# xkuubix/MonteCarlo-Gated-MIL

Measured on AMD Instinct MI355X. Metric: bags/sec × MCDO-samples (T=100) at N=2048,d=512; 1/2/4/8-GPU + %HBM roofline, higher is better.
Workload: dtype bf16

## Files before the change

montecarlo-gated-mil_amd/csrc/mcgmil_fused.hip:

```cpp
#define MCGMIL_KERNELS_TEMPLATES_ONLY
#include "../../include/mcgmil.h"
#include "mcgmil_kernels.h"
#include "mcgmil_error.h"
#include "mcgmil_fused.h"


namespace mcgmil {

__global__ __launch_bounds__(1024) void plan_regions_kernel(const int32_t* bag_off, int B, int T,
                                                            int cap, int32_t* region_off) {
    __shared__ int part[1024];
    const int tid = threadIdx.x;
    const int per = (B + 1023) / 1024;
    const int b0 = tid * per, b1 = b0 + per < B ? b0 + per : B;
    int sum = 0;
    for (int b = b0; b < b1; ++b) {
        const int ts = region_t_groups(bag_off[b + 1] - bag_off[b], T, cap);
        sum += (T + ts - 1) / ts;
    }
    part[tid] = sum;
    __syncthreads();
    for (int o = 1; o < 1024; o <<= 1) {
        const int v = tid >= o ? part[tid - o] : 0;
        __syncthreads();
        part[tid] += v;
        __syncthreads();
    }
    int run = part[tid] - sum;
    for (int b = b0; b < b1; ++b) {
        region_off[b] = run;
        const int ts = region_t_groups(bag_off[b + 1] - bag_off[b], T, cap);
        run += (T + ts - 1) / ts;
    }
    if (tid == 1023) region_off[B] = part[1023];
}

}

namespace mcgmil_detail {

long long fused_regions(const mcgmil::GateParams& gp, long long total_rows, int cap, bool estimate) {
    if (gp.uniform_rows > 0) {
        const int ts = mcgmil::region_t_groups(gp.uniform_rows, gp.T, cap);
        return (long long)gp.B * ((gp.T + ts - 1) / ts);
    }
    if (estimate) return (long long)gp.T * total_rows / cap;
    return (2ll * gp.T * total_rows + cap - 1) / cap + gp.B + 1;
}

namespace {

template <typename E, int PPW, int MAXC, bool ONE>
int launch(const mcgmil::GateParams& gp, long long total_rows, hipStream_t s) {
    auto* k = gp.clock ? &mcgmil::gate_fused_kernel<E, PPW, MAXC, ONE, true>
                       : &mcgmil::gate_fused_kernel<E, PPW, MAXC, ONE>;
    if (int rc = raise_lds_limit(reinterpret_cast<const void*>(k), "gate_fused_kernel LDS limit")) return rc;
    constexpr int cap = mcgmil::fused_cap<MAXC>();
    if (gp.uniform_rows <= 0) {
        hipLaunchKernelGGL(mcgmil::plan_regions_kernel, dim3(1), dim3(1024), 0, s, gp.bag_off, gp.B,
                           gp.T, cap, const_cast<int32_t*>(gp.region_off));
        hipError_t e = hipGetLastError();
        if (e != hipSuccess) return hip_fail(e, "plan_regions_kernel launch");
    }
    const long long grid = fused_regions(gp, total_rows, cap, false);
    if (grid == 0) return MCGMIL_OK;
    if (grid > 0x7fffffffll) return fail(MCGMIL_E_UNSUPPORTED, "too many regions for one launch");
    const size_t lds = mcgmil::fused_kernel_lds_bytes<E, MAXC>(gp.L);
    if (lds > 160 * 1024) return fail(MCGMIL_E_UNSUPPORTED, "fused kernel: L too large for its LDS");
    hipLaunchKernelGGL(k, dim3((unsigned)grid), dim3(mcgmil::kGateThreads), lds, s, gp);
    hipError_t e = hipGetLastError();
    return e == hipSuccess ? MCGMIL_OK : hip_fail(e, "gate_fused_kernel launch");
}

template <typename E, int MAXC>
int launch_maxc(const mcgmil::GateParams& gp, int ppw, bool one, long long total_rows, hipStream_t s) {
    if (ppw == 1) return one ? launch<E, 1, MAXC, true>(gp, total_rows, s) : launch<E, 1, MAXC, false>(gp, total_rows, s);
    return one ? launch<E, 2, MAXC, true>(gp, total_rows, s) : launch<E, 2, MAXC, false>(gp, total_rows, s);
}

}

int launch_gate_fused(const mcgmil::GateParams& gp, bool bf16, int ppw, int maxc, bool one,
                      long long total_rows, hipStream_t s) {
    if (bf16) return maxc == 2 ? launch_maxc<__bf16, 2>(gp, ppw, one, total_rows, s)
                               : launch_maxc<__bf16, 4>(gp, ppw, one, total_rows, s);
    return maxc == 2 ? launch_maxc<float, 2>(gp, ppw, one, total_rows, s)
                     : launch_maxc<float, 4>(gp, ppw, one, total_rows, s);
}

}
```

montecarlo-gated-mil_amd/csrc/mcgmil_kernels.h:

```cpp
#pragma once
#include "mcgmil_device.h"

namespace mcgmil {

struct GateParams {
    const void* H;
    long long ldh;
    const int32_t* bag_off;
    int B, T, L, D, C, G, P;
    long long total_samples;
    const void* Wp;
    uint32_t wp_bytes;
    const float* bv;
    const float* bu;
    const float* wa;
    const float* ba;
    float sf, sa;
    uint32_t thr_f, thr_a;
    uint32_t thrx_f;
    uint32_t k0, k1;
    uint32_t bag_base;
    int t_base;
    const uint32_t* bag_ids;
    const int32_t* tile_bag;
// ... 51 lines not shown
        Nb = p.uniform_rows;
        if (narrow) {
            const uint32_t r = (uint32_t)R, pb = (uint32_t)per_bag;
            bag = (int)(r / pb);
            const uint32_t local = r - (uint32_t)bag * pb;
            t = (int)(local / (uint32_t)Nb);
            n = (int)(local - (uint32_t)t * (uint32_t)Nb);
        } else {
            bag = (int)(R / per_bag);
            const long long local = R - (long long)bag * per_bag;
            t = (int)(local / Nb);
            n = (int)(local - (long long)t * Nb);
        }
        hrow = bag * Nb + n;
    } else if (R < p.total_samples) {
        if (p.tile_bag) {
            bag = p.tile_bag[R0 / BM];
            while ((long long)p.T * p.bag_off[bag + 1] <= R) ++bag;
        } else {
            bag = find_bag(p.bag_off, p.B, p.T, R);
        }
        const int ob = p.bag_off[bag];
        Nb = p.bag_off[bag + 1] - ob;
        const long long local = R - (long long)p.T * ob;
        if (narrow) {
            t = (int)((uint32_t)local / (uint32_t)Nb);
            n = (int)((uint32_t)local - (uint32_t)t * (uint32_t)Nb);
        } else {
            t = (int)(local / Nb);
            n = (int)(local - (long long)t * Nb);
        }
        hrow = ob + n;
    }
    int* ri = rinfo + kRowInfo * tid;
    ri[0] = hrow; ri[1] = t; ri[2] = n; ri[3] = bag; ri[4] = Nb;
    ri[5] = (int)(p.bag_ids ? p.bag_ids[bag] : p.bag_base + (uint32_t)bag);
}

#ifndef MCGMIL_KERNELS_TEMPLATES_ONLY
__global__ void plan_tiles_kernel(const int32_t* bag_off, int B, int T, long long total_samples,
                                  int BM, long long tiles, int32_t* tile_bag) {
    const long long i = (long long)blockIdx.x * blockDim.x + threadIdx.x;
    if (i >= tiles) return;
    const long long R = i * BM;
    tile_bag[i] = R < total_samples ? find_bag(bag_off, B, T, R) : 0;
}
#endif

__device__ __forceinline__ float gated_product_scaled(float ax, float by) {
    ax = fminf(fmaxf(ax, -43.280851226668903f), 43.280851226668903f);
    const float a = __builtin_amdgcn_exp2f(ax);
    const float b = __builtin_amdgcn_exp2f(by);
    const float ia = 1.0f + a;
    return (1.0f - a) * __builtin_amdgcn_rcpf(fmaf(ia, b, ia));
}

#ifndef MCGMIL_DIAG
#define MCGMIL_DIAG 0
#endif
#ifndef MCGMIL_PHILOX_ROUNDS
#define MCGMIL_PHILOX_ROUNDS 10
#endif

constexpr float kM2Log2e = -2.8853900817779268f;
constexpr float kMLog2e = -1.4426950408889634f;

struct HeadVec { f32x4 bv, bu, wa; };

template <int PPW>
__device__ __forceinline__ void load_head_vectors(const GateParams& p, int q0, int lane,
                                                  HeadVec (&hv)[PPW]) {
    const int DB = p.D >> 4;
#pragma unroll
    for (int jp = 0; jp < PPW; ++jp) {
        const int q = q0 + jp < p.P ? q0 + jp : p.P - 1;
        const int g = q / DB, db = q - g * DB;
        const int d0 = db * 16 + 4 * (lane >> 4);
        hv[jp].bv = *reinterpret_cast<const f32x4*>(p.bv + (size_t)g * p.D + d0) * kM2Log2e;
        hv[jp].bu = *reinterpret_cast<const f32x4*>(p.bu + (size_t)g * p.D + d0) * kMLog2e;
        hv[jp].wa = *reinterpret_cast<const f32x4*>(p.wa + (size_t)g * p.D + d0);
    }
}

template <int RT, int PPW, int MAXC, bool ONE_CLASS, int RTV = RT>
__device__ __forceinline__ void fold_pairs(const GateParams& p, const f32x4 (&acc)[RT][2 * PPW],
                                           int q0, int lane, float (&part)[MAXC][RT],
                                           const HeadVec* pre = nullptr) {
    const int DB = p.D >> 4;
    const float av_s = p.sf * kM2Log2e, au_s = p.sf * kMLog2e;
#pragma unroll
    for (int jp = 0; jp < PPW; ++jp) {
        const int q = q0 + jp;
        if (q >= p.P) break;
        const int g = q / DB, db = q - g * DB;
        const int d0 = db * 16 + 4 * (lane >> 4);
        f32x4 bvv, buv;
        f32x4 coef[MAXC];
        if (ONE_CLASS && pre) {
            bvv = pre[jp].bv;
            buv = pre[jp].bu;
            coef[0] = pre[jp].wa;
#pragma unroll
            for (int c = 1; c < MAXC; ++c) coef[c] = f32x4{0.f, 0.f, 0.f, 0.f};
        } else {
            bvv = *reinterpret_cast<const f32x4*>(p.bv + (size_t)g * p.D + d0);
            buv = *reinterpret_cast<const f32x4*>(p.bu + (size_t)g * p.D + d0);
            bvv *= kM2Log2e;
            buv *= kMLog2e;
#pragma unroll
            for (int c = 0; c < MAXC; ++c) {
                const int cc = ONE_CLASS ? g : c;
                const bool use = ONE_CLASS ? (c == 0) : ((c < p.C) && (p.G == 1 || c == g));
                const f32x4 w = *reinterpret_cast<const f32x4*>(p.wa + (size_t)(use ? cc : 0) * p.D + d0);
                coef[c] = use ? w : f32x4{0.f, 0.f, 0.f, 0.f};
            }
        }
#pragma unroll
        for (int rt = 0; rt < RTV; ++rt) {
#pragma unroll
            for (int v = 0; v < 4; ++v) {
                const float ax = fmaf(acc[rt][2 * jp][v], av_s, bvv[v]);
                const float by = fmaf(acc[rt][2 * jp + 1][v], au_s, buv[v]);
                if constexpr (ONE_CLASS) {
#if MCGMIL_DIAG & 8
                    part[0][rt] = fmaf(fmaf(ax, coef[0][v], by), ax, part[0][rt]);
                    continue;
#endif
                    const float a = __builtin_amdgcn_exp2f(fminf(fmaxf(ax, -43.280851226668903f),
                                                                 43.280851226668903f));
                    const float b = __builtin_amdgcn_exp2f(by);
                    const float ia = 1.0f + a;
                    const float r = __builtin_amdgcn_rcpf(fmaf(ia, b, ia));
                    part[0][rt] = fmaf(fmaf(-a, coef[0][v], coef[0][v]), r, part[0][rt]);
                } else {
                    const float pr = gated_product_scaled(ax, by);
#pragma unroll
                    for (int c = 0; c < MAXC; ++c) part[c][rt] = fmaf(pr, coef[c][v], part[c][rt]);
                }
            }
        }
    }
}

template <int BM, int MAXC>
__host__ __device__ constexpr int red_floats() { return kGateWaves * MAXC * 4 * BM; }

template <int BM, int MAXC, int ROWS = 16>
__device__ __forceinline__ void finish_scores(const GateParams& p, long long R0,
                                              float (&part)[MAXC][BM / ROWS], f32x4 zacc,
                                              bool zwave, float* red, float* zred,
                                              const int* rinfo, int one_class, int waves_per_gate,
                                              bool have_keep, bool keep, float* lg_out,
                                              float* z_out, long long obase) {
    constexpr int RT = BM / ROWS;
    constexpr int NG = 64 / ROWS;
    const int tid = threadIdx.x, lane = tid & 63, wave = tid >> 6;
    const int ncls = one_class < 0 ? MAXC : 1;
#pragma unroll
    for (int c = 0; c < MAXC; ++c) {
        if (c >= ncls) break;
        const int cls = one_class < 0 ? c : one_class;
        if (cls >= MAXC) break;
        float* dst = red + ((size_t)(wave * MAXC + cls) * NG + lane / ROWS) * BM + (lane % ROWS);
#pragma unroll
        for (int q = 0; q < RT; ++q) dst[ROWS * q] = part[c][q];
    }
    if (zwave && lane < 16) {
#pragma unroll
        for (int c = 0; c < MAXC; ++c) zred[c * BM + wave * 16 + lane] = zacc[c];
    }
    MCGMIL_STAMP(p, 5);
    __syncthreads();
    MCGMIL_STAMP(p, 6);
    const int r = wave * 16 + (lane & 15), c = lane >> 4;
    if (r >= BM || c >= p.C) return;
    const int* ri = rinfo + kRowInfo * r;
    if (ri[0] < 0) return;
    float s = 0.f;
    const int nw = waves_per_gate ? waves_per_gate : kGateWaves;
    for (int k = 0; k < nw; ++k) {
        const int w = waves_per_gate ? c * waves_per_gate + k : k;
        const float* src = red + (size_t)(w * MAXC + c) * NG * BM + r;
#pragma unroll
        for (int g = 0; g < NG; ++g) s += src[g * BM];
    }
    s += p.ba[c];
    const int t = ri[1], n = ri[2], bag = ri[3], Nb = ri[4];
    if (p.keep_att) {
        const size_t abase = (size_t)p.T * p.C * (size_t)p.bag_off[bag];
        keep = p.keep_att[abase + ((size_t)t * p.C + c) * Nb + n] != 0;
    } else if (!have_keep) {
        keep = attention_keep(p.k0, p.k1, (uint32_t)ri[5], (uint32_t)(p.t_base + t), (uint32_t)c,
                              (uint32_t)n, p.thr_a);
    }
    const size_t o = (size_t)(R0 + r - obase) * p.C + c;
    lg_out[o] = s * (keep ? p.sa : 0.f);
    z_out[o] = zred[c * BM + r] * p.sf;
}

constexpr int kSoftmaxRows = 16;

#ifndef MCGMIL_NT_A
#define MCGMIL_NT_A 1
#endif
__device__ __forceinline__ void store_a(float* dst, float v) {
#if MCGMIL_NT_A
    __builtin_nontemporal_store(v, dst);
#else
    *dst = v;
#endif
}

__device__ __forceinline__ void softmax_group(int ltid, bool active, int Nb, int C, const float* lg,
                                              const float* zz, float* Ao, float* Yo, float* sred) {
    const int tid = ltid, lane = ltid & 63, wave = ltid >> 6;
    if (Nb == 0) {
        if (active && tid < C) Yo[tid] = 0.f;
        return;
    }
    const int Nl = active ? Nb : 0;
    if (C == 2 && Nb <= 256 * kSoftmaxRows) {
        float (*sred2)[4] = reinterpret_cast<float (*)[4]>(sred);
        float e0[kSoftmaxRows], e1[kSoftmaxRows];
        float2 zr[kSoftmaxRows];
        float m0 = -INFINITY, m1 = -INFINITY;
#pragma unroll
        for (int k = 0; k < kSoftmaxRows; ++k) {
            const int n = tid + 256 * k;
            float2 l = make_float2(-INFINITY, -INFINITY);
            zr[k] = make_float2(0.f, 0.f);
            if (n < Nl) {
                l = *reinterpret_cast<const float2*>(lg + (size_t)n * 2);
                zr[k] = *reinterpret_cast<const float2*>(zz + (size_t)n * 2);
            }
            e0[k] = l.x;
            e1[k] = l.y;
            m0 = fmaxf(m0, e0[k]);
            m1 = fmaxf(m1, e1[k]);
        }
        m0 = wave_max(m0);
        m1 = wave_max(m1);
        if (lane == 0) { sred2[0][wave] = m0; sred2[1][wave] = m1; }
        __syncthreads();
        m0 = fmaxf(fmaxf(sred2[0][0], sred2[0][1]), fmaxf(sred2[0][2], sred2[0][3]));
        m1 = fmaxf(fmaxf(sred2[1][0], sred2[1][1]), fmaxf(sred2[1][2], sred2[1][3]));
        __syncthreads();
        float s0 = 0.f, y0 = 0.f, s1 = 0.f, y1 = 0.f;
#pragma unroll
        for (int k = 0; k < kSoftmaxRows; ++k) {
            const int n = tid + 256 * k;
            if (n < Nl) {
                const float2 z = zr[k];
                e0[k] = expf(e0[k] - m0);
                e1[k] = expf(e1[k] - m1);
                s0 += e0[k];
                s1 += e1[k];
                y0 = fmaf(e0[k], z.x, y0);
                y1 = fmaf(e1[k], z.y, y1);
            }
        }
        s0 = wave_sum(s0);
        y0 = wave_sum(y0);
        s1 = wave_sum(s1);
        y1 = wave_sum(y1);
        if (lane == 0) {
            sred2[0][wave] = s0; sred2[1][wave] = y0; sred2[2][wave] = s1; sred2[3][wave] = y1;
        }
        __syncthreads();
        s0 = (sred2[0][0] + sred2[0][1]) + (sred2[0][2] + sred2[0][3]);
        y0 = (sred2[1][0] + sred2[1][1]) + (sred2[1][2] + sred2[1][3]);
        s1 = (sred2[2][0] + sred2[2][1]) + (sred2[2][2] + sred2[2][3]);
        y1 = (sred2[3][0] + sred2[3][1]) + (sred2[3][2] + sred2[3][3]);
        __syncthreads();
        const float inv0 = 1.0f / s0, inv1 = 1.0f / s1;
        if (Ao) {
            float* Ao1 = Ao + Nb;
#pragma unroll
            for (int k = 0; k < kSoftmaxRows; ++k) {
// ... 101 lines not shown
template <> struct Raw<__bf16> { uint4 v; };
template <> struct Raw<float> { f32x4 lo, hi; };
__device__ __forceinline__ Raw<__bf16> load_raw(const __bf16* p) {
    Raw<__bf16> r; r.v = *reinterpret_cast<const uint4*>(p); return r;
}
__device__ __forceinline__ Raw<float> load_raw(const float* p) {
    Raw<float> r;
    r.lo = *reinterpret_cast<const f32x4*>(p);
    r.hi = *reinterpret_cast<const f32x4*>(p + 4);
    return r;
}
__device__ __forceinline__ void store_masked(const Raw<__bf16>& h, uint32_t kb, __bf16* dst) {
    uint4 v = h.v;
    v.x &= ((kb & 1u) ? 0x0000FFFFu : 0u) | ((kb & 2u) ? 0xFFFF0000u : 0u);
    v.y &= ((kb & 4u) ? 0x0000FFFFu : 0u) | ((kb & 8u) ? 0xFFFF0000u : 0u);
    v.z &= ((kb & 16u) ? 0x0000FFFFu : 0u) | ((kb & 32u) ? 0xFFFF0000u : 0u);
    v.w &= ((kb & 64u) ? 0x0000FFFFu : 0u) | ((kb & 128u) ? 0xFFFF0000u : 0u);
    *reinterpret_cast<uint4*>(dst) = v;
}
__device__ __forceinline__ void store_masked(const Raw<float>& h, uint32_t kb, float* dst) {
    f32x4 a = h.lo, b = h.hi;
    a.x = (kb & 1u) ? a.x : 0.f;   a.y = (kb & 2u) ? a.y : 0.f;
    a.z = (kb & 4u) ? a.z : 0.f;   a.w = (kb & 8u) ? a.w : 0.f;
    b.x = (kb & 16u) ? b.x : 0.f;  b.y = (kb & 32u) ? b.y : 0.f;
    b.z = (kb & 64u) ? b.z : 0.f;  b.w = (kb & 128u) ? b.w : 0.f;
    *reinterpret_cast<f32x4*>(dst) = a;
    *reinterpret_cast<f32x4*>(dst + 4) = b;
}

__device__ __forceinline__ void store_dropped(const Raw<__bf16>& h, uint4 o, uint32_t thrx,
                                              uint32_t inval, __bf16* dst) {
    uint4 v = h.v;
    v.x = __builtin_amdgcn_bitop3_b32(v.x, drop_mask16x2_flipped(o.x, thrx), inval, 0x10);
    v.y = __builtin_amdgcn_bitop3_b32(v.y, drop_mask16x2(o.y, thrx), inval, 0x10);
    v.z = __builtin_amdgcn_bitop3_b32(v.z, drop_mask16x2_flipped(o.z, thrx), inval, 0x10);
    v.w = __builtin_amdgcn_bitop3_b32(v.w, drop_mask16x2(o.w, thrx), inval, 0x10);
    *reinterpret_cast<uint4*>(dst) = v;
}
__device__ __forceinline__ uint32_t keep_lo(uint32_t m) { return ~(uint32_t)((int32_t)(m << 16) >> 16); }
__device__ __forceinline__ uint32_t keep_hi(uint32_t m) { return ~(uint32_t)((int32_t)m >> 16); }
__device__ __forceinline__ void store_dropped(const Raw<float>& h, uint4 o, uint32_t thrx,
                                              uint32_t inval, float* dst) {
    const uint32_t m0 = drop_mask16x2_flipped(o.x, thrx) | inval, m1 = drop_mask16x2(o.y, thrx) | inval;
    const uint32_t m2 = drop_mask16x2_flipped(o.z, thrx) | inval, m3 = drop_mask16x2(o.w, thrx) | inval;
    f32x4 a = h.lo, b = h.hi;
    a.x = __uint_as_float(__float_as_uint(a.x) & keep_lo(m0));
    a.y = __uint_as_float(__float_as_uint(a.y) & keep_hi(m0));
    a.z = __uint_as_float(__float_as_uint(a.z) & keep_lo(m1));
    a.w = __uint_as_float(__float_as_uint(a.w) & keep_hi(m1));
    b.x = __uint_as_float(__float_as_uint(b.x) & keep_lo(m2));
    b.y = __uint_as_float(__float_as_uint(b.y) & keep_hi(m2));
    b.z = __uint_as_float(__float_as_uint(b.z) & keep_lo(m3));
    b.w = __uint_as_float(__float_as_uint(b.w) & keep_hi(m3));
    *reinterpret_cast<f32x4*>(dst) = a;
    *reinterpret_cast<f32x4*>(dst + 4) = b;
}

constexpr int kPipeBM = 128;
#ifndef MCGMIL_VPM
#define MCGMIL_VPM 2
#endif
constexpr int VPM = MCGMIL_VPM;
#ifndef MCGMIL_SCHED
#define MCGMIL_SCHED 0
#endif
constexpr int HD = 2;
template <typename E>
__host__ __device__ constexpr int pipe_slots() { return 2; }

template <typename E, int MAXC>
__host__ __device__ constexpr size_t pipe_lds_bytes() {
    return (size_t)pipe_slots<E>() * kPipeBM * 32 * sizeof(E) + (size_t)red_floats<kPipeBM, MAXC>() * 4 +
           (size_t)MAXC * kPipeBM * 4 + (size_t)kRowInfo * kPipeBM * 4;
}

template <typename E>
__device__ __forceinline__ void load_classifier_lds(__amdgpu_buffer_rsrc_t wrs, uint32_t zsoff, int KS, E* zw) {
    for (int i = threadIdx.x; i < KS * 64; i += kGateThreads)
        *reinterpret_cast<f32x4*>(zw + (size_t)i * 8) = __builtin_bit_cast(
            f32x4, __builtin_amdgcn_raw_buffer_load_b128(wrs, (uint32_t)i * 8u * (uint32_t)sizeof(E), zsoff, 0));
}

template <typename E, int PPW, int MAXC, bool REPLAY, bool ONE_CLASS, bool EARLY_HV = true,
          bool ZL = false, bool ZLOAD = true, int RTV = kPipeBM / 16>
__device__ __forceinline__ void pipe_tile(const GateParams& p, long long R0, E* Xs, float* red,
                                          float* zred, const int* rinfo, float* lg_out,
                                          float* z_out, long long obase, E* zw = nullptr) {
    constexpr int BM = kPipeBM;
    constexpr int RT = BM / 16;
    constexpr int NJ = 2 * PPW;
    constexpr int SLOT = RT * 64 * 8;
    const int tid = threadIdx.x, lane = tid & 63, wave = tid >> 6;
    const int KS = p.L >> 5;

    const int* ri = rinfo + kRowInfo * (wave * 16 + (lane & 15));
    const int hrow = ri[0];
    const bool valid = hrow >= 0;
    const int kq = lane >> 4;
    const E* hsrc = reinterpret_cast<const E*>(p.H) + (size_t)(valid ? hrow : 0) * p.ldh + kq * 8;
    const uint32_t cn = (uint32_t)ri[2], ct = (uint32_t)(p.t_base + ri[1]), cb = (uint32_t)ri[5];
    const uint8_t* kfe = REPLAY ? p.keep_feat + (size_t)(valid ? R0 + wave * 16 + (lane & 15) : 0) *
                                                    (p.L >> 3) + kq
                                : nullptr;

    const uint32_t inval = valid ? 0u : 0xFFFFFFFFu;
    auto stage = [&](int s, const Raw<E>& h, E* slot) {
        if constexpr (REPLAY) {
            const uint32_t kb = kfe[(size_t)(s < KS ? s : KS - 1) * 4];
            store_masked(h, kb & ~inval, slot + tid * 8);
        } else {
#if MCGMIL_DIAG & 4
            const uint4 o = make_uint4(cn * 0x9E3779B9u + (uint32_t)s, ct ^ cb, cn + ct, (uint32_t)s * 77u);
#else
            const uint4 o = philox4x32_10<true, MCGMIL_PHILOX_ROUNDS>((uint32_t)(s * 4 + kq), cn, ct, cb, p.k0, p.k1);
#endif
            store_dropped(h, o, p.thrx_f, inval, slot + tid * 8);
        }
    };

    const __amdgpu_buffer_rsrc_t wrs = make_rsrc(p.Wp, p.wp_bytes);
    const uint32_t tile_bytes = (uint32_t)KS * 512u * (uint32_t)sizeof(E);
    constexpr uint32_t kStepBytes = 512u * (uint32_t)sizeof(E);
    const int q0 = __builtin_amdgcn_readfirstlane(wave) * PPW;
    uint32_t wsoff[NJ];
#pragma unroll
    for (int j = 0; j < NJ; ++j) {
        int q = q0 + (j >> 1);
        q = q < p.P ? q : p.P - 1;
        wsoff[j] = (uint32_t)(2 * q + (j & 1)) * tile_bytes;
    }
    const uint32_t zsoff = (uint32_t)(2 * p.P) * tile_bytes;
    const uint32_t lane_b = (uint32_t)lane * 8u * (uint32_t)sizeof(E);
    auto wfrag = [&](uint32_t soff) { return load_frag_buf<E>(wrs, lane_b, soff); };

    f32x4 acc[RT][NJ];
#pragma unroll
    for (int rt = 0; rt < RT; ++rt)
#pragma unroll
        for (int j = 0; j < NJ; ++j) acc[rt][j] = f32x4{0.f, 0.f, 0.f, 0.f};
    f32x4 zacc = {0.f, 0.f, 0.f, 0.f};

    auto kstep = [&](int s, const E* cur, E* nxt, const Frag<E> (&w)[NJ], const Frag<E>& z,
                     Frag<E> (&wn)[NJ], Frag<E>& zn, const Raw<E>& h, Raw<E>& hn) {
        const int s1 = s + 1 < KS ? s + 1 : KS - 1;
        const int sh = s + HD < KS ? s + HD : KS - 1;
#if MCGMIL_DIAG & 2
#pragma unroll
        for (int j = 0; j < NJ; ++j) wn[j] = w[j];
        zn = z;
#else
#pragma unroll
        for (int j = 0; j < NJ; ++j) wn[j] = wfrag(wsoff[j] + (uint32_t)s1 * kStepBytes);
        if constexpr (!ZL) zn = wfrag(zsoff + (uint32_t)s1 * kStepBytes);
#endif
#if MCGMIL_DIAG & 1
        hn = h;
#else
        if (RTV == RT || wave < RTV) hn = load_raw(hsrc + (size_t)sh * 32);
#endif
#pragma unroll
        for (int rt = 0; rt < RTV; ++rt) {
            const Frag<E> x = load_frag(cur + (size_t)(rt * 64 + lane) * 8);
#pragma unroll
            for (int j = 0; j < NJ; ++j) acc[rt][j] = mma(w[j], x, acc[rt][j]);
        }
        const Frag<E> xz = load_frag(cur + (size_t)tid * 8);
        if constexpr (ZL) zacc = mma(load_frag(zw + (size_t)(s * 64 + lane) * 8), xz, zacc);
        else zacc = mma(z, xz, zacc);
        if (RTV == RT || wave < RTV) stage(s + 1, h, nxt);
        if constexpr (sizeof(E) == 2 && PPW == 2) {
#if MCGMIL_SCHED == 1
            __builtin_amdgcn_sched_group_barrier(0x020, NJ + 2, 0);
            __builtin_amdgcn_sched_group_barrier(0x100, 3, 0);
#pragma unroll
            for (int rt = 0; rt < RT; ++rt) {
#pragma unroll
                for (int j = 0; j < NJ; ++j) {
                    __builtin_amdgcn_sched_group_barrier(0x008, 1, 0);
                    __builtin_amdgcn_sched_group_barrier(0x002, VPM, 0);
                }
                if (rt + 2 < RT) __builtin_amdgcn_sched_group_barrier(0x100, 1, 0);
            }
            __builtin_amdgcn_sched_group_barrier(0x008, 1, 0);
            __builtin_amdgcn_sched_group_barrier(0x002, VPM, 0);
#else
#pragma unroll
            for (int i = 0; i < RTV * NJ + 1; ++i) {
                __builtin_amdgcn_sched_group_barrier(0x008, 1, 0);
                __builtin_amdgcn_sched_group_barrier(0x002, VPM, 0);
            }
#endif
        }
#if MCGMIL_DIAG & 128
        asm volatile("s_waitcnt lgkmcnt(0)" ::: "memory");
#else
        __syncthreads();
#endif
    };

    constexpr bool kEarlyHV = EARLY_HV && ONE_CLASS && sizeof(E) == 2;
    HeadVec hvec[PPW];
    {
        Frag<E> wA[NJ], wB[NJ], zA, zB;
        Raw<E> hA{}, hB{};
        if (RTV == RT || wave < RTV) {
            hA = load_raw(hsrc);
            hB = load_raw(hsrc + 32);
        }
#pragma unroll
        for (int j = 0; j < NJ; ++j) wA[j] = wfrag(wsoff[j]);
        if constexpr (ZL) {
            if constexpr (ZLOAD) load_classifier_lds<E>(wrs, zsoff, KS, zw);
        } else {
            zA = wfrag(zsoff);
        }
        if (RTV == RT || wave < RTV) stage(0, hA, Xs);
        __syncthreads();
        MCGMIL_STAMP(p, 2);

        if constexpr (kEarlyHV) load_head_vectors<PPW>(p, q0, lane, hvec);
        kstep(0, Xs, Xs + SLOT, wA, zA, wB, zB, hB, hA);
        kstep(1, Xs + SLOT, Xs, wB, zB, wA, zA, hA, hB);
#if MCGMIL_DIAG & 16
        if (KS > 1000)
#endif
        for (int s = 2; s < KS; s += 2) {
            kstep(s, Xs, Xs + SLOT, wA, zA, wB, zB, hB, hA);
            kstep(s + 1, Xs + SLOT, Xs, wB, zB, wA, zA, hA, hB);
        }
    }
    MCGMIL_STAMP(p, 3);

    float part[MAXC][RT];
#pragma unroll
    for (int c = 0; c < MAXC; ++c)
#pragma unroll
        for (int rt = 0; rt < RT; ++rt) part[c][rt] = 0.f;
    fold_pairs<RT, PPW, MAXC, ONE_CLASS, RTV>(p, acc, q0, lane, part, kEarlyHV ? hvec : nullptr);
    MCGMIL_STAMP(p, 4);
    const int one_class = ONE_CLASS ? (q0 < p.P ? q0 / (p.D >> 4) : MAXC) : -1;
    finish_scores<BM, MAXC>(p, R0, part, zacc, true, red, zred, rinfo, one_class,
                            ONE_CLASS ? (p.D >> 4) / PPW : 0, false, true, lg_out, z_out, obase);
    MCGMIL_STAMP(p, 7);
}

#ifndef MCGMIL_XCD_TILES
#define MCGMIL_XCD_TILES 1
#endif
__device__ __forceinline__ long long xcd_tile(unsigned b, unsigned n, int bags) {
#if MCGMIL_XCD_TILES
    const unsigned x = b & 7u, q = n >> 3, r = n & 7u;
    const unsigned l = (x < r ? x * (q + 1) : r * (q + 1) + (x - r) * q) + (b >> 3);
    return (long long)(bags >= 8 ? l : b);
#else
    (void)n;
    (void)bags;
    return (long long)b;
#endif
}

template <typename E, int PPW, int MAXC, bool REPLAY, bool ONE_CLASS, bool PROBE = false, int RTV = kPipeBM / 16>
__global__ __launch_bounds__(kGateThreads) void gate_pipe_kernel(const GateParams p) {
    extern __shared__ __attribute__((aligned(16))) unsigned char smem[];
    constexpr int BM = kPipeBM;
    E* Xs = reinterpret_cast<E*>(smem);
    float* red = reinterpret_cast<float*>(smem + (size_t)pipe_slots<E>() * BM * 32 * sizeof(E));
    float* zred = red + red_floats<BM, MAXC>();
    int* rinfo = reinterpret_cast<int*>(zred + MAXC * BM);
    const long long R0 = RTV == BM / 16 ? xcd_tile(blockIdx.x, gridDim.x, p.B) * BM
                                        : p.tile_row0 + (long long)blockIdx.x * (16 * RTV);

    if constexpr (PROBE) clock_probe(p, 0);
    MCGMIL_STAMP(p, 0);
    fill_row_table<BM, 16 * RTV>(p, R0, rinfo);
    __syncthreads();
    MCGMIL_STAMP(p, 1);
    pipe_tile<E, PPW, MAXC, REPLAY, ONE_CLASS, true, false, true, RTV>(p, R0, Xs, red, zred, rinfo, p.logits,
                                                                       p.zz, 0);
    if constexpr (PROBE) clock_probe(p, 1);
}

#ifndef MCGMIL_FUSED_XCD
#define MCGMIL_FUSED_XCD 1
#endif
#ifndef MCGMIL_FUSED_EARLY_HV
#define MCGMIL_FUSED_EARLY_HV 0
#endif
#ifndef MCGMIL_FUSED_NMAJOR
#define MCGMIL_FUSED_NMAJOR 1
#endif
#ifndef MCGMIL_FUSED_CAP
#define MCGMIL_FUSED_CAP 4096
#endif
template <int MAXC>
__host__ __device__ constexpr int fused_cap() { return MAXC <= 2 ? MCGMIL_FUSED_CAP : MCGMIL_FUSED_CAP / 4; }

template <typename E, int MAXC>
__host__ __device__ constexpr size_t fused_lds_bytes() {
    return pipe_lds_bytes<E, MAXC>() + (size_t)kRowInfo * kPipeBM * 4
           + (size_t)2 * fused_cap<MAXC>() * MAXC * 4
           + (size_t)2 * 16 * 4 + 64;
}

#ifndef MCGMIL_FUSED_ZL
#define MCGMIL_FUSED_ZL 1
#endif
template <typename E>
__host__ __device__ constexpr bool fused_zl() { return MCGMIL_FUSED_ZL && sizeof(E) == 2; }
template <typename E, int MAXC>
__host__ __device__ constexpr size_t fused_kernel_lds_bytes(int L) {
    return fused_lds_bytes<E, MAXC>() + (fused_zl<E>() ? (size_t)(L / 32) * 512 * sizeof(E) : 0);
}

__host__ __device__ inline int region_t_groups(int Nb, int T, int cap) {
    if (Nb <= 0) return T;
    if (Nb > cap) return 1;
    const int ts = cap / Nb;
    return ts < T ? ts : T;
}

struct Region {
    int bag, t0, t1, Nb, ob;
    int ntiles;
    long long S, rows;
};

__device__ __forceinline__ int region_tile(const Region& rg, int i) {
#if MCGMIL_FUSED_NMAJOR
    const int G = rg.t1 - rg.t0;
    if (G > 1 && rg.Nb % kPipeBM == 0) return (i % G) * (rg.Nb / kPipeBM) + i / G;
#endif
    return i;
}

__device__ __forceinline__ GateParams reload_kernarg_params(const GateParams& p) {
#if __HIP_DEVICE_COMPILE__
    typedef __attribute__((address_space(4))) const GateParams* KernargParams;
    KernargParams q = (KernargParams)__builtin_amdgcn_kernarg_segment_ptr();
    asm volatile("" : "+s"(q));
    return *q;
#else
    return p;
#endif
}

__device__ __forceinline__ bool decode_region(const GateParams& p, int g, int cap, Region& rg) {
    int b, j, ts;
    if (p.uniform_rows > 0) {
        ts = p.region_t;
        const int rpb = (p.T + ts - 1) / ts;
        if (MCGMIL_FUSED_XCD && (p.B & 7) == 0) {
            const int k = g >> 3;
            b = 8 * (k / rpb) + (g & 7);
            j = k - (k / rpb) * rpb;
        } else {
            b = g / rpb;
            j = g - b * rpb;
        }
        if (b >= p.B) return false;
    } else {
        if (g >= p.region_off[p.B]) return false;
        b = find_bag(p.region_off, p.B, 1, g);
        j = g - p.region_off[b];
        ts = region_t_groups(p.bag_off[b + 1] - p.bag_off[b], p.T, cap);
    }
    rg.bag = b;
    rg.ob = p.bag_off[b];
    rg.Nb = p.bag_off[b + 1] - rg.ob;
    rg.t0 = j * ts;
    rg.t1 = rg.t0 + ts < p.T ? rg.t0 + ts : p.T;
    rg.S = (long long)p.T * rg.ob + (long long)rg.t0 * rg.Nb;
    rg.rows = (long long)(rg.t1 - rg.t0) * rg.Nb;
    rg.ntiles = (int)((rg.rows + kPipeBM - 1) / kPipeBM);
    return true;
}

template <int BM>
__device__ __forceinline__ void fill_row_table_region(const GateParams& p, const Region& rg,
                                                      long long R0, int* rinfo) {
    const int tid = threadIdx.x;
    if (tid >= BM) return;
    const long long rho = R0 + tid - rg.S;
    int hrow = -1, t = 0, n = 0;
    if (rho < rg.rows) {
        const uint32_t r = (uint32_t)rho;
        const uint32_t tt = r / (uint32_t)rg.Nb;
        n = (int)(r - tt * (uint32_t)rg.Nb);
        t = rg.t0 + (int)tt;
        hrow = rg.ob + n;
    }
    int* ri = rinfo + kRowInfo * tid;
    ri[0] = hrow; ri[1] = t; ri[2] = n; ri[3] = rg.bag; ri[4] = rg.Nb;
    ri[5] = (int)(p.bag_ids ? p.bag_ids[rg.bag] : p.bag_base + (uint32_t)rg.bag);
}


template <typename E, int PPW, int MAXC, bool ONE_CLASS, bool PROBE = false>
__global__ __launch_bounds__(kGateThreads) void gate_fused_kernel(const GateParams p) {
    extern __shared__ __attribute__((aligned(16))) unsigned char smem[];
    constexpr int BM = kPipeBM;
    constexpr int CAP = fused_cap<MAXC>();
    E* Xs = reinterpret_cast<E*>(smem);
    float* red = reinterpret_cast<float*>(smem + (size_t)pipe_slots<E>() * BM * 32 * sizeof(E));
    float* zred = red + red_floats<BM, MAXC>();
    int* rinfo = reinterpret_cast<int*>(zred + MAXC * BM);
    float* slg = reinterpret_cast<float*>(rinfo + 2 * kRowInfo * BM);
    float* szz = slg + CAP * MAXC;
    float* sred = szz + CAP * MAXC;

#if MCGMIL_DIAG & 64
    {
        const long long R0 = (long long)blockIdx.x * BM;
        fill_row_table<BM>(p, R0, rinfo);
        __syncthreads();
        pipe_tile<E, PPW, MAXC, false, ONE_CLASS>(p, R0, Xs, red, zred, rinfo, p.logits, p.zz, 0);
        return;
    }
#endif
    Region rg;
    if (!decode_region(p, (int)blockIdx.x, CAP, rg)) return;
    if constexpr (PROBE) clock_probe(p, 0);
    const int ntiles = (int)((rg.rows + BM - 1) / BM);
    Region* srg = reinterpret_cast<Region*>(sred + 32);
    if (threadIdx.x == 0) *srg = rg;
    __syncthreads();
    E* zw = reinterpret_cast<E*>(smem + fused_lds_bytes<E, MAXC>());
    if constexpr (fused_zl<E>())
        load_classifier_lds<E>(make_rsrc(p.Wp, p.wp_bytes), (uint32_t)(2 * p.P) * (uint32_t)(p.L >> 5) * 512u *
                                   (uint32_t)sizeof(E), p.L >> 5, zw);
    for (int i = 0; i < ntiles; ++i) {
        Region* qr = srg;
        asm volatile("" : "+v"(qr));
        const GateParams pt = reload_kernarg_params(p);
        int* ri = rinfo + (i & 1) * kRowInfo * BM;
        MCGMIL_STAMP(pt, 0);
        {
            const Region r = *qr;
            fill_row_table_region<BM>(pt, r, r.S + (long long)region_tile(r, i) * BM, ri);
        }
        __syncthreads();
        MCGMIL_STAMP(pt, 1);
        const Region r = *qr;
        const bool lds = r.Nb <= CAP;
        pipe_tile<E, PPW, MAXC, false, ONE_CLASS, MCGMIL_FUSED_EARLY_HV, fused_zl<E>(), false>(
            pt, r.S + (long long)region_tile(r, i) * BM, Xs, red, zred, ri, lds ? slg : pt.logits,
            lds ? szz : pt.zz, lds ? r.S : 0, zw);
    }
    __syncthreads();
#if MCGMIL_DIAG & 32
    if (ntiles >= 0) return;
#endif
    rg = *srg;
    const bool in_lds = rg.Nb <= CAP;

    const int G = rg.t1 - rg.t0;
    const int half = threadIdx.x >> 8, ltid = threadIdx.x & 255;
    for (int j0 = 0; j0 < G; j0 += 2) {
        const bool act = j0 + half < G;
        const int j = act ? j0 + half : j0;
        const long long row0 = (long long)j * rg.Nb;
        const float* lgj = in_lds ? slg + row0 * p.C : p.logits + (rg.S + row0) * p.C;
        const float* zzj = in_lds ? szz + row0 * p.C : p.zz + (rg.S + row0) * p.C;
        float* Ao = p.A ? p.A + (size_t)p.T * p.C * rg.ob + (size_t)(rg.t0 + j) * p.C * rg.Nb : nullptr;
        float* Yo = p.Y + ((size_t)rg.bag * p.T + rg.t0 + j) * p.C;
        softmax_group(ltid, act, rg.Nb, p.C, lgj, zzj, Ao, Yo, sred + half * 16);
    }
    if constexpr (PROBE) clock_probe(p, 1);
}

template <int BM>
__host__ __device__ constexpr int gate_row_info_ints() { return kRowInfo * BM; }

template <typename E, int BM, int MAXC>
__host__ __device__ constexpr size_t gate_lds_bytes(int L) {
    const size_t tile = (size_t)BM * L * sizeof(E), red = (size_t)red_floats<BM, MAXC>() * 4;
    return (tile > red ? tile : red) + (size_t)MAXC * BM * 4 + (size_t)gate_row_info_ints<BM>() * 4;
}

template <typename E, int BM, int PPW, int MAXC>
__global__ __launch_bounds__(kGateThreads) void gate_scores_kernel(const GateParams p) {
    extern __shared__ __attribute__((aligned(16))) unsigned char smem[];
    constexpr int RT = BM / 16;
    constexpr int NJ = 2 * PPW;
    const int tid = threadIdx.x;
    const int lane = tid & 63;
    const int wave = tid >> 6;
    const int L = p.L;
    const int KS = L >> 5;
    const int LC = L >> 3;

    E* Xs = reinterpret_cast<E*>(smem);
    float* red = reinterpret_cast<float*>(smem);
    const size_t tile_bytes = (size_t)BM * L * sizeof(E), red_bytes = (size_t)red_floats<BM, MAXC>() * 4;
    float* zred = reinterpret_cast<float*>(smem + (tile_bytes > red_bytes ? tile_bytes : red_bytes));
    int* rinfo = reinterpret_cast<int*>(zred + MAXC * BM);
    const long long R0 = (long long)blockIdx.x * BM;

    fill_row_table<BM>(p, R0, rinfo);
    __syncthreads();

    {
        const E* H = reinterpret_cast<const E*>(p.H);
        const int items = BM * LC;
        for (int i = tid; i < items; i += kGateThreads) {
            const int blk = i >> 6, slot = i & 63;
            const int rt = blk / KS, ks = blk - rt * KS;
            const int r = rt * 16 + (slot & 15);
            const int kc = ks * 4 + (slot >> 4);
            E* dst = Xs + ((size_t)blk * 64 + slot) * 8;
            const int* ri = rinfo + kRowInfo * r;
            const int hrow = ri[0];
            if (hrow < 0) {
                store_zero8(dst);
                continue;
            }
            uint32_t kb;
            if (p.keep_feat) {
                kb = p.keep_feat[(size_t)(R0 + r) * LC + kc];
            } else {
                const uint4 o = philox4x32_10((uint32_t)kc, (uint32_t)ri[2],
                                              (uint32_t)(p.t_base + ri[1]), (uint32_t)ri[5],
                                              p.k0, p.k1);
                kb = keep_byte(o, p.thr_f);
            }
            load_masked(H + (size_t)hrow * p.ldh + (size_t)kc * 8, kb, dst);
        }
    }
    __syncthreads();

    const E* Wp = reinterpret_cast<const E*>(p.Wp);
    const int pairs_per_pass = kGateWaves * PPW;
    const int npass = (p.P + pairs_per_pass - 1) / pairs_per_pass;
    const size_t tile_elems = (size_t)KS * 512;

    float part[MAXC][RT];
#pragma unroll
    for (int c = 0; c < MAXC; ++c)
#pragma unroll
        for (int rt = 0; rt < RT; ++rt) part[c][rt] = 0.f;
    f32x4 zacc = {0.f, 0.f, 0.f, 0.f};
    const bool zwave = wave < RT;

    for (int pass = 0; pass < npass; ++pass) {
        const int q0 = pass * pairs_per_pass + wave * PPW;
        const bool active = q0 < p.P;
        const bool doz = (pass == 0) && zwave;
        if (!active && !doz) continue;

        f32x4 acc[RT][NJ];
#pragma unroll
// ... 196 lines not shown
```

Baseline: 893,300.

## Add affine fused-kernel path with per-region LDS constants instead of row tables

For uniform bag sizes that are multiples of the tile height and fit in the region cap, the fused kernel now computes row, sample and bag indices from a per-region constant block in LDS (tile descriptors, bag counter, biases, class per wave). This replaces the per-tile row-info table fill and its barrier. Head vectors are also pre-scaled into LDS once per block. The goal is to cut per-tile index bookkeeping, global loads and synchronisation, at the cost of an extra kernel variant and a larger LDS footprint.

```diff
diff --git a/montecarlo-gated-mil_amd/csrc/mcgmil_fused.hip b/montecarlo-gated-mil_amd/csrc/mcgmil_fused.hip
--- a/montecarlo-gated-mil_amd/csrc/mcgmil_fused.hip
+++ b/montecarlo-gated-mil_amd/csrc/mcgmil_fused.hip
@@ -52,10 +52,13 @@
 
 template <typename E, int PPW, int MAXC, bool ONE>
 int launch(const mcgmil::GateParams& gp, long long total_rows, hipStream_t s) {
-    auto* k = gp.clock ? &mcgmil::gate_fused_kernel<E, PPW, MAXC, ONE, true>
-                       : &mcgmil::gate_fused_kernel<E, PPW, MAXC, ONE>;
+    constexpr int cap = mcgmil::fused_cap<MAXC>();
+    const bool affine = mcgmil::fused_affine(gp.uniform_rows, cap);
+    auto* k = affine ? (gp.clock ? &mcgmil::gate_fused_kernel<E, PPW, MAXC, ONE, true>
+                                 : &mcgmil::gate_fused_kernel<E, PPW, MAXC, ONE>)
+                     : (gp.clock ? &mcgmil::gate_fused_table_kernel<E, PPW, MAXC, ONE, true>
+                                 : &mcgmil::gate_fused_table_kernel<E, PPW, MAXC, ONE>);
     if (int rc = raise_lds_limit(reinterpret_cast<const void*>(k), "gate_fused_kernel LDS limit")) return rc;
-    constexpr int cap = mcgmil::fused_cap<MAXC>();
     if (gp.uniform_rows <= 0) {
         hipLaunchKernelGGL(mcgmil::plan_regions_kernel, dim3(1), dim3(1024), 0, s, gp.bag_off, gp.B,
                            gp.T, cap, const_cast<int32_t*>(gp.region_off));
diff --git a/montecarlo-gated-mil_amd/csrc/mcgmil_kernels.h b/montecarlo-gated-mil_amd/csrc/mcgmil_kernels.h
--- a/montecarlo-gated-mil_amd/csrc/mcgmil_kernels.h
+++ b/montecarlo-gated-mil_amd/csrc/mcgmil_kernels.h
@@ -157,6 +157,41 @@
     }
 }
 
+struct Region {
+    int bag, t0, t1, Nb, ob;
+    int ntiles;
+    long long S, rows;
+};
+
+constexpr int kFusedTiles = 32;
+constexpr int kFusedHv = 256;
+struct alignas(16) FusedConst {
+    Region rg;
+    uint32_t bagctr;
+    int pad0;
+    float ba[4];
+    int cls[8];
+    int pad1[8];
+    int4 tile[kFusedTiles];
+    float hv[3][kFusedHv];
+};
+
+#ifndef MCGMIL_FUSED_HV_LDS
+#define MCGMIL_FUSED_HV_LDS 1
+#endif
+template <int PPW>
+__device__ __forceinline__ void load_head_vectors_lds(const FusedConst* fc, int P, int q0, int lane,
+                                                      HeadVec (&hv)[PPW]) {
+#pragma unroll
+    for (int jp = 0; jp < PPW; ++jp) {
+        const int q = q0 + jp < P ? q0 + jp : P - 1;
+        const int d = 16 * q + 4 * (lane >> 4);
+        hv[jp].bv = *reinterpret_cast<const f32x4*>(fc->hv[0] + d);
+        hv[jp].bu = *reinterpret_cast<const f32x4*>(fc->hv[1] + d);
+        hv[jp].wa = *reinterpret_cast<const f32x4*>(fc->hv[2] + d);
+    }
+}
+
 template <int RT, int PPW, int MAXC, bool ONE_CLASS, int RTV = RT>
 __device__ __forceinline__ void fold_pairs(const GateParams& p, const f32x4 (&acc)[RT][2 * PPW],
                                            int q0, int lane, float (&part)[MAXC][RT],
@@ -167,8 +202,9 @@
     for (int jp = 0; jp < PPW; ++jp) {
         const int q = q0 + jp;
         if (q >= p.P) break;
-        const int g = q / DB, db = q - g * DB;
-        const int d0 = db * 16 + 4 * (lane >> 4);
+        const int col = 16 * q + 4 * (lane >> 4);
+        const int g = ONE_CLASS ? 0 : q / DB;
+        const int d0 = col - g * p.D;
         f32x4 bvv, buv;
         f32x4 coef[MAXC];
         if (ONE_CLASS && pre) {
@@ -178,8 +214,8 @@
 #pragma unroll
             for (int c = 1; c < MAXC; ++c) coef[c] = f32x4{0.f, 0.f, 0.f, 0.f};
         } else {
-            bvv = *reinterpret_cast<const f32x4*>(p.bv + (size_t)g * p.D + d0);
-            buv = *reinterpret_cast<const f32x4*>(p.bu + (size_t)g * p.D + d0);
+            bvv = *reinterpret_cast<const f32x4*>(p.bv + col);
+            buv = *reinterpret_cast<const f32x4*>(p.bu + col);
             bvv *= kM2Log2e;
             buv *= kMLog2e;
 #pragma unroll
@@ -220,13 +256,14 @@
 template <int BM, int MAXC>
 __host__ __device__ constexpr int red_floats() { return kGateWaves * MAXC * 4 * BM; }
 
-template <int BM, int MAXC, int ROWS = 16>
+template <int BM, int MAXC, int ROWS = 16, bool AFFINE = false>
 __device__ __forceinline__ void finish_scores(const GateParams& p, long long R0,
                                               float (&part)[MAXC][BM / ROWS], f32x4 zacc,
                                               bool zwave, float* red, float* zred,
                                               const int* rinfo, int one_class, int waves_per_gate,
                                               bool have_keep, bool keep, float* lg_out,
-                                              float* z_out, long long obase) {
+                                              float* z_out, long long obase,
+                                              const FusedConst* fc = nullptr, int tile = 0) {
     constexpr int RT = BM / ROWS;
     constexpr int NG = 64 / ROWS;
     const int tid = threadIdx.x, lane = tid & 63, wave = tid >> 6;
@@ -249,8 +286,24 @@
     MCGMIL_STAMP(p, 6);
     const int r = wave * 16 + (lane & 15), c = lane >> 4;
     if (r >= BM || c >= p.C) return;
-    const int* ri = rinfo + kRowInfo * r;
-    if (ri[0] < 0) return;
+    int t, n, bag, Nb;
+    uint32_t bagc;
+    size_t orow;
+    float bias;
+    if constexpr (AFFINE) {
+        const int4 tl = fc->tile[tile];
+        t = tl.x, n = tl.y + r, bag = fc->rg.bag, Nb = fc->rg.Nb;
+        bagc = fc->bagctr;
+        orow = (size_t)(tl.z + r);
+        bias = fc->ba[c];
+    } else {
+        const int* ri = rinfo + kRowInfo * r;
+        if (ri[0] < 0) return;
+        t = ri[1], n = ri[2], bag = ri[3], Nb = ri[4];
+        bagc = (uint32_t)ri[5];
+        orow = (size_t)(R0 + r - obase);
+        bias = p.ba[c];
+    }
     float s = 0.f;
     const int nw = waves_per_gate ? waves_per_gate : kGateWaves;
     for (int k = 0; k < nw; ++k) {
@@ -259,16 +312,15 @@
 #pragma unroll
         for (int g = 0; g < NG; ++g) s += src[g * BM];
     }
-    s += p.ba[c];
-    const int t = ri[1], n = ri[2], bag = ri[3], Nb = ri[4];
+    s += bias;
     if (p.keep_att) {
         const size_t abase = (size_t)p.T * p.C * (size_t)p.bag_off[bag];
         keep = p.keep_att[abase + ((size_t)t * p.C + c) * Nb + n] != 0;
     } else if (!have_keep) {
-        keep = attention_keep(p.k0, p.k1, (uint32_t)ri[5], (uint32_t)(p.t_base + t), (uint32_t)c,
+        keep = attention_keep(p.k0, p.k1, bagc, (uint32_t)(p.t_base + t), (uint32_t)c,
                               (uint32_t)n, p.thr_a);
     }
-    const size_t o = (size_t)(R0 + r - obase) * p.C + c;
+    const size_t o = orow * p.C + c;
     lg_out[o] = s * (keep ? p.sa : 0.f);
     z_out[o] = zred[c * BM + r] * p.sf;
 }
@@ -536,10 +588,11 @@
 }
 
 template <typename E, int PPW, int MAXC, bool REPLAY, bool ONE_CLASS, bool EARLY_HV = true,
-          bool ZL = false, bool ZLOAD = true, int RTV = kPipeBM / 16>
+          bool ZL = false, bool ZLOAD = true, int RTV = kPipeBM / 16, bool AFFINE = false>
 __device__ __forceinline__ void pipe_tile(const GateParams& p, long long R0, E* Xs, float* red,
                                           float* zred, const int* rinfo, float* lg_out,
-                                          float* z_out, long long obase, E* zw = nullptr) {
+                                          float* z_out, long long obase, E* zw = nullptr,
+                                          const FusedConst* fc = nullptr, int tile = 0) {
     constexpr int BM = kPipeBM;
     constexpr int RT = BM / 16;
     constexpr int NJ = 2 * PPW;
@@ -547,12 +600,23 @@
     const int tid = threadIdx.x, lane = tid & 63, wave = tid >> 6;
     const int KS = p.L >> 5;
 
-    const int* ri = rinfo + kRowInfo * (wave * 16 + (lane & 15));
-    const int hrow = ri[0];
-    const bool valid = hrow >= 0;
+    int hrow;
+    uint32_t cn, ct, cb;
+    if constexpr (AFFINE) {
+        static_assert(!REPLAY, "the affine rows have no replay masks");
+        const int4 tl = fc->tile[tile];
+        cn = (uint32_t)(tl.y + wave * 16 + (lane & 15));
+        hrow = fc->rg.ob + (int)cn;
+        ct = (uint32_t)(p.t_base + tl.x);
+        cb = fc->bagctr;
+    } else {
+        const int* ri = rinfo + kRowInfo * (wave * 16 + (lane & 15));
+        hrow = ri[0];
+        cn = (uint32_t)ri[2], ct = (uint32_t)(p.t_base + ri[1]), cb = (uint32_t)ri[5];
+    }
+    const bool valid = AFFINE || hrow >= 0;
     const int kq = lane >> 4;
     const E* hsrc = reinterpret_cast<const E*>(p.H) + (size_t)(valid ? hrow : 0) * p.ldh + kq * 8;
-    const uint32_t cn = (uint32_t)ri[2], ct = (uint32_t)(p.t_base + ri[1]), cb = (uint32_t)ri[5];
     const uint8_t* kfe = REPLAY ? p.keep_feat + (size_t)(valid ? R0 + wave * 16 + (lane & 15) : 0) *
                                                     (p.L >> 3) + kq
                                 : nullptr;
@@ -690,11 +754,16 @@
     for (int c = 0; c < MAXC; ++c)
 #pragma unroll
         for (int rt = 0; rt < RT; ++rt) part[c][rt] = 0.f;
-    fold_pairs<RT, PPW, MAXC, ONE_CLASS, RTV>(p, acc, q0, lane, part, kEarlyHV ? hvec : nullptr);
+    constexpr bool kLdsHV = MCGMIL_FUSED_HV_LDS && AFFINE && ONE_CLASS && !kEarlyHV;
+    if constexpr (kLdsHV) load_head_vectors_lds<PPW>(fc, p.P, q0, lane, hvec);
+    fold_pairs<RT, PPW, MAXC, ONE_CLASS, RTV>(p, acc, q0, lane, part, kEarlyHV || kLdsHV ? hvec : nullptr);
     MCGMIL_STAMP(p, 4);
-    const int one_class = ONE_CLASS ? (q0 < p.P ? q0 / (p.D >> 4) : MAXC) : -1;
-    finish_scores<BM, MAXC>(p, R0, part, zacc, true, red, zred, rinfo, one_class,
-                            ONE_CLASS ? (p.D >> 4) / PPW : 0, false, true, lg_out, z_out, obase);
+    int one_class = -1;
+    if constexpr (ONE_CLASS && AFFINE) one_class = __builtin_amdgcn_readfirstlane(fc->cls[wave]);
+    else if constexpr (ONE_CLASS) one_class = q0 < p.P ? q0 / (p.D >> 4) : MAXC;
+    finish_scores<BM, MAXC, 16, AFFINE>(p, R0, part, zacc, true, red, zred, rinfo, one_class,
+                                        ONE_CLASS ? (p.D >> 4) / PPW : 0, false, true, lg_out, z_out,
+                                        obase, fc, tile);
     MCGMIL_STAMP(p, 7);
 }
 
@@ -753,7 +822,12 @@
 __host__ __device__ constexpr size_t fused_lds_bytes() {
     return pipe_lds_bytes<E, MAXC>() + (size_t)kRowInfo * kPipeBM * 4
            + (size_t)2 * fused_cap<MAXC>() * MAXC * 4
-           + (size_t)2 * 16 * 4 + 64;
+           + (size_t)2 * 16 * 4 + sizeof(FusedConst);
+}
+static_assert(kFusedTiles * kPipeBM >= MCGMIL_FUSED_CAP, "FusedConst::tile holds a whole region");
+
+__host__ __device__ inline bool fused_affine(int uniform_rows, int cap) {
+    return uniform_rows > 0 && uniform_rows % kPipeBM == 0 && uniform_rows <= cap;
 }
 
 #ifndef MCGMIL_FUSED_ZL
@@ -772,12 +846,6 @@
     const int ts = cap / Nb;
     return ts < T ? ts : T;
 }
-
-struct Region {
-    int bag, t0, t1, Nb, ob;
-    int ntiles;
-    long long S, rows;
-};
 
 __device__ __forceinline__ int region_tile(const Region& rg, int i) {
 #if MCGMIL_FUSED_NMAJOR
@@ -849,8 +917,38 @@
 }
 
 
-template <typename E, int PPW, int MAXC, bool ONE_CLASS, bool PROBE = false>
-__global__ __launch_bounds__(kGateThreads) void gate_fused_kernel(const GateParams p) {
+template <int PPW, int MAXC, bool ONE_CLASS>
+__device__ __forceinline__ void fill_fused_const(const GateParams& p, const Region& rg, FusedConst* fc) {
+    const int tid = threadIdx.x;
+    if (tid == 0) {
+        fc->rg = rg;
+        fc->bagctr = p.bag_ids ? p.bag_ids[rg.bag] : p.bag_base + (uint32_t)rg.bag;
+    }
+    if (tid < MAXC) fc->ba[tid] = tid < p.C ? p.ba[tid] : 0.f;
+    if (tid < kGateWaves) {
+        const int q0 = tid * PPW, DB = p.D >> 4;
+        int g = 0;
+        while ((g + 1) * DB <= q0) ++g;
+        fc->cls[tid] = ONE_CLASS && q0 < p.P ? g : MAXC;
+    }
+    if (tid < rg.ntiles && tid < kFusedTiles) {
+        const int G = rg.t1 - rg.t0, nbt = rg.Nb / kPipeBM;
+        const int dv = MCGMIL_FUSED_NMAJOR ? G : nbt;
+        int qt = 0;
+        while ((qt + 1) * dv <= tid) ++qt;
+        const int rem = tid - qt * dv;
+        const int tg = MCGMIL_FUSED_NMAJOR ? rem : qt, nb = MCGMIL_FUSED_NMAJOR ? qt : rem;
+        fc->tile[tid] = make_int4(rg.t0 + tg, nb * kPipeBM, tg * rg.Nb + nb * kPipeBM, 0);
+    }
+    if (ONE_CLASS && tid < 16 * p.P && tid < kFusedHv) {
+        fc->hv[0][tid] = p.bv[tid] * kM2Log2e;
+        fc->hv[1][tid] = p.bu[tid] * kMLog2e;
+        fc->hv[2][tid] = p.wa[tid];
+    }
+}
+
+template <typename E, int PPW, int MAXC, bool ONE_CLASS, bool PROBE, bool AFFINE>
+__device__ __forceinline__ void fused_region(const GateParams& p) {
     extern __shared__ __attribute__((aligned(16))) unsigned char smem[];
     constexpr int BM = kPipeBM;
     constexpr int CAP = fused_cap<MAXC>();
@@ -861,6 +959,7 @@
     float* slg = reinterpret_cast<float*>(rinfo + 2 * kRowInfo * BM);
     float* szz = slg + CAP * MAXC;
     float* sred = szz + CAP * MAXC;
+    FusedConst* fc = reinterpret_cast<FusedConst*>(sred + 32);
 
 #if MCGMIL_DIAG & 64
     {
@@ -875,37 +974,45 @@
     if (!decode_region(p, (int)blockIdx.x, CAP, rg)) return;
     if constexpr (PROBE) clock_probe(p, 0);
     const int ntiles = (int)((rg.rows + BM - 1) / BM);
-    Region* srg = reinterpret_cast<Region*>(sred + 32);
-    if (threadIdx.x == 0) *srg = rg;
+    Region* srg = &fc->rg;
+    if constexpr (AFFINE) fill_fused_const<PPW, MAXC, ONE_CLASS>(p, rg, fc);
+    else if (threadIdx.x == 0) *srg = rg;
     __syncthreads();
     E* zw = reinterpret_cast<E*>(smem + fused_lds_bytes<E, MAXC>());
     if constexpr (fused_zl<E>())
         load_classifier_lds<E>(make_rsrc(p.Wp, p.wp_bytes), (uint32_t)(2 * p.P) * (uint32_t)(p.L >> 5) * 512u *
                                    (uint32_t)sizeof(E), p.L >> 5, zw);
     for (int i = 0; i < ntiles; ++i) {
-        Region* qr = srg;
-        asm volatile("" : "+v"(qr));
         const GateParams pt = reload_kernarg_params(p);
-        int* ri = rinfo + (i & 1) * kRowInfo * BM;
-        MCGMIL_STAMP(pt, 0);
-        {
+        if constexpr (AFFINE) {
+            MCGMIL_STAMP(pt, 0);
+            MCGMIL_STAMP(pt, 1);
+            pipe_tile<E, PPW, MAXC, false, ONE_CLASS, MCGMIL_FUSED_EARLY_HV, fused_zl<E>(), false, BM / 16, true>(
+                pt, 0, Xs, red, zred, nullptr, slg, szz, 0, zw, fc, i);
+        } else {
+            Region* qr = srg;
+            asm volatile("" : "+v"(qr));
+            int* ri = rinfo + (i & 1) * kRowInfo * BM;
+            MCGMIL_STAMP(pt, 0);
+            {
+                const Region r = *qr;
+                fill_row_table_region<BM>(pt, r, r.S + (long long)region_tile(r, i) * BM, ri);
+            }
+            __syncthreads();
+            MCGMIL_STAMP(pt, 1);
             const Region r = *qr;
-            fill_row_table_region<BM>(pt, r, r.S + (long long)region_tile(r, i) * BM, ri);
-        }
-        __syncthreads();
-        MCGMIL_STAMP(pt, 1);
-        const Region r = *qr;
-        const bool lds = r.Nb <= CAP;
-        pipe_tile<E, PPW, MAXC, false, ONE_CLASS, MCGMIL_FUSED_EARLY_HV, fused_zl<E>(), false>(
-            pt, r.S + (long long)region_tile(r, i) * BM, Xs, red, zred, ri, lds ? slg : pt.logits,
-            lds ? szz : pt.zz, lds ? r.S : 0, zw);
+            const bool lds = r.Nb <= CAP;
+            pipe_tile<E, PPW, MAXC, false, ONE_CLASS, MCGMIL_FUSED_EARLY_HV, fused_zl<E>(), false>(
+                pt, r.S + (long long)region_tile(r, i) * BM, Xs, red, zred, ri, lds ? slg : pt.logits,
+                lds ? szz : pt.zz, lds ? r.S : 0, zw);
+        }
     }
     __syncthreads();
 #if MCGMIL_DIAG & 32
     if (ntiles >= 0) return;
 #endif
     rg = *srg;
-    const bool in_lds = rg.Nb <= CAP;
+    const bool in_lds = AFFINE || rg.Nb <= CAP;
 
     const int G = rg.t1 - rg.t0;
     const int half = threadIdx.x >> 8, ltid = threadIdx.x & 255;
@@ -920,6 +1027,16 @@
         softmax_group(ltid, act, rg.Nb, p.C, lgj, zzj, Ao, Yo, sred + half * 16);
     }
     if constexpr (PROBE) clock_probe(p, 1);
+}
+
+template <typename E, int PPW, int MAXC, bool ONE_CLASS, bool PROBE = false>
+__global__ __launch_bounds__(kGateThreads) void gate_fused_kernel(const GateParams p) {
+    fused_region<E, PPW, MAXC, ONE_CLASS, PROBE, true>(p);
+}
+
+template <typename E, int PPW, int MAXC, bool ONE_CLASS, bool PROBE = false>
+__global__ __launch_bounds__(kGateThreads) void gate_fused_table_kernel(const GateParams p) {
+    fused_region<E, PPW, MAXC, ONE_CLASS, PROBE, false>(p);
 }
 
 template <int BM>
```

New measurement: 934,500, median of 6. 1.05x the previous value.
